# bifurcation/fourq

Hardware: NVIDIA B200
Metric: curve4q_variable_base_dh_scalar_mults_per_s (higher is better)
Workload: dtype u32

## Files before the change

### fourq_b200/csrc/codec.cuh

```cuda
#pragma once
#include "point.cuh"

#define FQ_ST_OK 0
#define FQ_ST_RESERVED_BIT 1
#define FQ_ST_NONCANONICAL 2
#define FQ_ST_QUIRK_T0 3
#define FQ_ST_NOT_ON_CURVE 4
#define FQ_ST_NEUTRAL 5

FQ_FN u32 pt_sign(const fp2& x) {
  u32 nz = x.re.v[0] | x.re.v[1] | x.re.v[2] | x.re.v[3];
  return (nz != 0) ? (x.re.v[3] >> 30) : (x.im.v[3] >> 30);
}

FQ_FN void pt_encode(const fp2& x, const fp2& y, u32* out) {
  FQ_UNROLL
  for (int i = 0; i < 4; i++) { out[i] = y.re.v[i]; out[4 + i] = y.im.v[i]; }
  out[7] |= pt_sign(x) << 31;
}

template <bool SPEC = false> FQ_FN u32 pt_decode(const u32* in, fp2& x, fp2& y) {
  u32 st = FQ_ST_OK;
  if (in[3] >> 31) st = FQ_ST_RESERVED_BIT;
  u32 s = in[7] >> 31;
  y.re = fp_set(in[0], in[1], in[2], in[3] & FQ_P3);
  y.im = fp_set(in[4], in[5], in[6], in[7] & FQ_P3);
  u32 y0p = in[0] & in[1] & in[2] & (in[3] | 0x80000000u);
  u32 y1p = in[4] & in[5] & in[6] & (in[7] | 0x80000000u);
  if (st == FQ_ST_OK && (y0p == 0xffffffffu || y1p == 0xffffffffu)) st = FQ_ST_NONCANONICAL;

  fp2 y2 = fp2_sqr_c(y);
  fp2 u = fp2_sub(y2, fp2_one());
  const fp2 dy2 = fp2_mul_c(curve_d(), y2);
  fp2 v = fp2_add(dy2, fp2_one());
  fpb V0 = fp_prep(v.re), V1 = fp_prep(v.im);
  fp t0 = fp_add(fp_mul_prep(u.re, V0), fp_mul_prep(u.im, V1));
  fp t1 = fp_sub(fp_mul_prep(u.im, V0), fp_mul_prep(u.re, V1));
  fp t2 = fp_add(fp_sqr(v.re), fp_sqr(v.im));
  fp t3 = fp_add(fp_sqr(t0), fp_sqr(t1));
  t3 = fp_mul(fp_invsqrt_c(t3), t3);
  fp t = fp_dbl(fp_add(t0, t3));
  if (SPEC) { if (fp_is_zero(t)) t = fp_dbl(fp_sub(t0, t3)); }
  else if (st == FQ_ST_OK && fp_is_zero(t)) st = FQ_ST_QUIRK_T0;
  fpb T2 = fp_prep(t2);
  fp a = fp_invsqrt_c(fp_mul(fp_mul_prep(fp_sqr(t2), T2), t));
  fp at2 = fp_mul_prep(a, T2);
  fp b = fp_mul(at2, t);
  fp x0 = fp_half(b);
  fp x1 = fp_mul(at2, t1);
  bool same = fp_eq_canon(fp_canon(t), fp_canon(fp_mul_prep(fp_sqr(b), T2)));
  u32 msw = same ? 0u : 0xffffffffu;
  x.re = fp_canon(fp_select(msw, x1, x0));
  x.im = fp_canon(fp_select(msw, x0, x1));
  u32 mneg = (pt_sign(x) != s) ? 0xffffffffu : 0u;
  x = fp2_canon(fp2_select(mneg, fp2_neg(x), x));
  y = fp2_canon(y);
  const fp2 x2 = fp2_sqr_c(x), x2c = fp2_conj(x2);
  bool on1 = fp2_eq(fp2_sub(y2, x2), fp2_add(fp2_one(), fp2_mul_c(dy2, x2)));
  fp2 xc = fp2_canon(fp2_conj(x));
  bool on2 = fp2_eq(fp2_sub(y2, x2c), fp2_add(fp2_one(), fp2_mul_c(dy2, x2c)));
  x = fp2_select(on1 ? 0xffffffffu : 0u, x, xc);
  if (st == FQ_ST_OK && !(on1 | on2)) st = FQ_ST_NOT_ON_CURVE;
  return st;
}
```

### fourq_b200/csrc/endo.cuh

```cuda
#pragma once
#include "dh.cuh"

FQ_FN fp2 endo_ctau() { return fp2_set(fp_set(0xebce74c3u, 0x74dcd57cu, 0x3afad20cu, 0x1964de2cu), fp_set(0x00000012u, 0x00000000u, 0x0000000cu, 0x00000000u)); }
FQ_FN fp2 endo_ctaudual() { return fp2_set(fp_set(0xdecdf034u, 0x9ecaa6d9u, 0x23058652u, 0x4aa740ebu), fp_set(0x00000011u, 0x00000000u, 0xfffffff4u, 0x7fffffffu)); }
FQ_FN fp2 endo_cphi0() { return fp2_set(fp_set(0xfffffff7u, 0xffffffffu, 0x00000005u, 0x00000000u), fp_set(0xef66f81au, 0x4f65536cu, 0x9182c329u, 0x2553a075u)); }
FQ_FN fp2 endo_cphi1() { return fp2_set(fp_set(0x00000007u, 0x00000000u, 0x00000005u, 0x00000000u), fp_set(0xe28296f9u, 0x334d90e9u, 0xc50c62cfu, 0x62c8caa0u)); }
FQ_FN fp2 endo_cphi2() { return fp2_set(fp_set(0x00000015u, 0x00000000u, 0x0000000fu, 0x00000000u), fp_set(0x4f1df391u, 0x2c2cb715u, 0x6c9b5c98u, 0x78df262bu)); }
FQ_FN fp2 endo_cphi3() { return fp2_set(fp_set(0x00000003u, 0x00000000u, 0x00000002u, 0x00000000u), fp_set(0xa7962ea4u, 0x92440457u, 0x1d76342au, 0x5084c649u)); }
FQ_FN fp2 endo_cphi4() { return fp2_set(fp_set(0x00000003u, 0x00000000u, 0x00000003u, 0x00000000u), fp_set(0x3aec6855u, 0xa1098c92u, 0xa7962ea4u, 0x12440457u)); }
FQ_FN fp2 endo_cphi5() { return fp2_set(fp_set(0x0000000fu, 0x00000000u, 0x0000000au, 0x00000000u), fp_set(0xc5052df3u, 0x669b21d3u, 0x8a18c59eu, 0x45919541u)); }
FQ_FN fp2 endo_cphi6() { return fp2_set(fp_set(0x00000018u, 0x00000000u, 0x00000012u, 0x00000000u), fp_set(0x8a0a5be7u, 0xcd3643a7u, 0x14318b3cu, 0x0b232a83u)); }
FQ_FN fp2 endo_cphi7() { return fp2_set(fp_set(0x00000023u, 0x00000000u, 0x00000018u, 0x00000000u), fp_set(0x5f48781au, 0x66c18303u, 0x99e2ea1au, 0x3963bc1cu)); }
FQ_FN fp2 endo_cphi8() { return fp2_set(fp_set(0x000000f0u, 0x00000000u, 0x000000aau, 0x00000000u), fp_set(0x2b5d0ef0u, 0x44e25158u, 0x0316cbe5u, 0x1f529f86u)); }
FQ_FN fp2 endo_cphi9() { return fp2_set(fp_set(0x00000befu, 0x00000000u, 0x00000870u, 0x00000000u), fp_set(0x976e2505u, 0x014d3e48u, 0xfe00375bu, 0x0fd52e9cu)); }
FQ_FN fp2 endo_cpsi1() { return fp2_set(fp_set(0x67e346efu, 0xedf07f47u, 0x83d54a02u, 0x2af99e9au), fp_set(0x0000013au, 0x00000000u, 0x000000deu, 0x00000000u)); }
FQ_FN fp2 endo_cpsi2() { return fp2_set(fp_set(0x00000143u, 0x00000000u, 0x000000e4u, 0x00000000u), fp_set(0x0e03f372u, 0x4c7deb77u, 0x99a81f03u, 0x21b8d07bu)); }
FQ_FN fp2 endo_cpsi3() { return fp2_set(fp_set(0x00000009u, 0x00000000u, 0x00000006u, 0x00000000u), fp_set(0x75e73a61u, 0x3a6e6abeu, 0x1d7d6906u, 0x4cb26f16u)); }
FQ_FN fp2 endo_cpsi4() { return fp2_set(fp_set(0xfffffff6u, 0xffffffffu, 0xfffffff9u, 0x7fffffffu), fp_set(0x8a18c59eu, 0xc5919541u, 0xe28296f9u, 0x334d90e9u)); }

struct pt3 { fp2 X, Y, Z; };

#if defined(FQ_ENDO_CALLS) && !defined(FQ_HOSTSIM)
#define FQ_ENDO_FN FQ_CALL
#else
#define FQ_ENDO_FN FQ_FN
#endif

FQ_FN fp2 fp2_two_sqr(const fp2& z) { return fp2_dbl(fp2_sqr_c(z)); }

FQ_ENDO_FN pt3 endo_tau(pt3 P) {
  fp2 A = fp2_sqr_c(P.X), B = fp2_sqr_c(P.Y);
  fp2 C = fp2_add(A, B), D = fp2_sub(A, B);
  pt3 R;
  R.X = fp2_mul_c(fp2_mul_c(fp2_mul_c(endo_ctau(), P.X), P.Y), D);
  R.Y = fp2_neg(fp2_mul_c(fp2_add(fp2_two_sqr(P.Z), D), C));
  R.Z = fp2_mul_c(C, D);
  return R;
}
FQ_ENDO_FN ptR1 endo_tau_dual(pt3 P) {
  fp2 A = fp2_sqr_c(P.X), B = fp2_sqr_c(P.Y);
  fp2 C = fp2_add(A, B);
  ptR1 R;
  R.Ta = fp2_sub(B, A);
  fp2 D = fp2_sub(fp2_two_sqr(P.Z), R.Ta);
  R.Tb = fp2_mul_c(fp2_mul_c(endo_ctaudual(), P.X), P.Y);
  R.X = fp2_mul_c(R.Tb, C); R.Y = fp2_mul_c(R.Ta, D); R.Z = fp2_mul_c(D, C);
  return R;
}
FQ_ENDO_FN pt3 endo_upsilon(pt3 P) {
  fp2 A = fp2_mul_c(fp2_mul_c(endo_cphi0(), P.X), P.Y);
  fp2 B = fp2_mul_c(P.Y, P.Z);
  fp2 C = fp2_sqr_c(P.Y), D = fp2_sqr_c(P.Z);
  fp2 F = fp2_sqr_c(D), G = fp2_sqr_c(B), H = fp2_sqr_c(C);
  fp2 I = fp2_mul_c(endo_cphi1(), B);
  fp2 J = fp2_add(C, fp2_mul_c(endo_cphi2(), D));
  fp2 K = fp2_add(fp2_add(fp2_mul_c(endo_cphi8(), G), H), fp2_mul_c(endo_cphi9(), F));
  pt3 R;
  R.X = fp2_conj(fp2_mul_c(fp2_mul_c(A, K), fp2_mul_c(fp2_add(I, J), fp2_sub(I, J))));
  fp2 L = fp2_add(C, fp2_mul_c(endo_cphi4(), D));
  fp2 M = fp2_mul_c(endo_cphi3(), B);
  fp2 Nn = fp2_mul_c(fp2_add(L, M), fp2_sub(L, M));
  fp2 Y2 = fp2_add(fp2_add(H, fp2_mul_c(endo_cphi6(), G)), fp2_mul_c(endo_cphi7(), F));
  R.Y = fp2_conj(fp2_mul_c(fp2_mul_c(fp2_mul_c(endo_cphi5(), D), Nn), Y2));
  R.Z = fp2_conj(fp2_mul_c(fp2_mul_c(B, K), Nn));
  return R;
}
FQ_ENDO_FN pt3 endo_chi(pt3 P) {
  fp2 A = fp2_conj(P.X), B = fp2_conj(P.Y);
  fp2 C = fp2_sqr_c(fp2_conj(P.Z));
  fp2 D = fp2_sqr_c(A);
  fp2 G = fp2_mul_c(B, fp2_add(D, fp2_mul_c(endo_cpsi2(), C)));
  fp2 H = fp2_neg(fp2_add(D, fp2_mul_c(endo_cpsi4(), C)));
  pt3 R;
  R.X = fp2_mul_c(fp2_mul_c(fp2_mul_c(endo_cpsi1(), A), C), H);
  R.Y = fp2_mul_c(G, fp2_add(D, fp2_mul_c(endo_cpsi3(), C)));
  R.Z = fp2_mul_c(G, H);
  return R;
}
FQ_FN pt3 pt3_of(const ptR1& P) { pt3 R; R.X = P.X; R.Y = P.Y; R.Z = P.Z; return R; }
FQ_FN ptR1 endo_phi(const ptR1& P) { return endo_tau_dual(endo_upsilon(endo_tau(pt3_of(P)))); }
FQ_FN ptR1 endo_psi(const ptR1& P) { return endo_tau_dual(endo_chi(endo_tau(pt3_of(P)))); }

FQ_CALL u64 endo_mulhi_256(u32 l0, u32 l1, u32 l2, u32 l3, u32 l4, u32 l5, u32 l6, scal m) {
  const u32 L[7] = {l0, l1, l2, l3, l4, l5, l6};
  u32 c0 = 0, c1 = 0, c2 = 0, out8 = 0, out9 = 0;
  FQ_UNROLL
  for (int k = 0; k < 10; k++) {
    FQ_UNROLL
    for (int i = 0; i < 7; i++) {
      const int j = k - i;
      if (j >= 0 && j < 8) { c0 = mad_lo_cc(L[i], m.v[j], c0); c1 = madc_hi_cc(L[i], m.v[j], c1); c2 = addc(c2, 0); }
    }
    if (k == 8) out8 = c0;
    if (k == 9) out9 = c0;
    c0 = c1; c1 = c2; c2 = 0;
  }
  return ((u64)out9 << 32) | out8;
}

struct scal4 { u64 v[4]; };

FQ_FN scal4 endo_decompose(const scal& m) {
  const u64 B1[4] = {0x0906ff27e0a0a196ull, 0xec9c179d3dd5d260ull, 0x07426031ecc8030full, 0xf7b08c66794619afull};
  const u64 B2[4] = {0x1d495bea84fcc2d4ull, 0xffffffffffffffffull, 0x0000000000000001ull, 0x25dbc5bc8dd167d0ull};
  const u64 B3[4] = {0x17abad1d231f0302ull, 0x02c4211ae388da51ull, 0xd1b2de3676d83b61ull, 0x0a9e6f44c02ecd97ull};
  const u64 B4[4] = {0x136e340a9108c83full, 0x3122df2dc3e0ff32ull, 0xf975b60fd557564bull, 0xe72af7876921f516ull};
  const u64 C[4] = {0x72482c5251a4559cull, 0x59f95b0add276f6cull, 0x7dd2d17c4625fa78ull, 0x6bc57def56ce8877ull};
  const u64 CP[4] = {0x85b6605ce2ad1ddbull, 0x8b1c3a38a1086e9eull, 0x7748878c1b7d50c3ull, 0x52f07576bff07d8dull};
  u64 t1 = endo_mulhi_256(0x9d1a7d4fu, 0x259686e0u, 0xe6a6bd66u, 0xf75682acu, 0xea2be5dfu, 0xfc5bb5c5u, 0x00000007u, m);
  u64 t2 = endo_mulhi_256(0xdd627afbu, 0xd1ba1d84u, 0x0f468d8du, 0x2bd23558u, 0xaa6c0f8au, 0x8fd4b04cu, 0x00000003u, m);
  u64 t3 = endo_mulhi_256(0x678c203cu, 0x9b291a33u, 0x65dca902u, 0xc42bd6c9u, 0x0bffbaf6u, 0xd038bf8du, 0x00000000u, m);
  u64 t4 = endo_mulhi_256(0x77e7fdc0u, 0x12e5666bu, 0x14983d82u, 0x81cbdc37u, 0xa22d8410u, 0x1b073877u, 0x00000003u, m);
  scal4 a;
  FQ_UNROLL
  for (int j = 0; j < 4; j++) {
    u64 x = (j == 0) ? (((u64)m.v[1] << 32) | m.v[0]) : 0ull;
    a.v[j] = x - t1 * B1[j] - t2 * B2[j] - t3 * B3[j] - t4 * B4[j];
  }
  u64 odd = 0ull - ((a.v[0] + C[0]) & 1ull);
  scal4 v;
  FQ_UNROLL
  for (int j = 0; j < 4; j++) v.v[j] = a.v[j] + ((C[j] & odd) | (CP[j] & ~odd));
  return v;
}

FQ_FN u32 endo_recode(const scal4& vin, scal& S) {
  u64 v0s = vin.v[0] >> 1, v1 = vin.v[1], v2 = vin.v[2], v3 = vin.v[3];
  FQ_UNROLL
  for (int w = 0; w < 8; w++) S.v[w] = 0;
  FQ_NOUNROLL
  for (int w = 0; w < 8; w++) {
    u32 word = 0;
    FQ_UNROLL
    for (int n = 0; n < 8; n++) {
      u32 b1 = (u32)(v0s & 1ull);
      v0s >>= 1;
      u32 e1 = (u32)(v1 & 1ull), e2 = (u32)(v2 & 1ull), e3 = (u32)(v3 & 1ull);
      word |= ((b1 << 3) | e1 | (e2 << 1) | (e3 << 2)) << (4 * n);
      u32 nb1 = b1 ^ 1u;
      v1 = (v1 >> 1) + (u64)(nb1 & e1); v2 = (v2 >> 1) + (u64)(nb1 & e2); v3 = (v3 >> 1) + (u64)(nb1 & e3);
    }
    FQ_UNROLL
    for (int i = 0; i < 7; i++) S.v[i] = S.v[i + 1];
    S.v[7] = word;
  }
  return (u32)(v1 + 2ull * v2 + 4ull * v3);
}
FQ_FN void endo_next_digit(scal& s, u32& idx, u32& neg) {
  u32 nib = s.v[7] >> 28;
  neg = (nib >> 3) - 1;
  idx = nib & 7;
  FQ_UNROLL
  for (int i = 7; i > 0; i--) s.v[i] = shl_pair(s.v[i - 1], s.v[i], 4);
  s.v[0] <<= 4;
}

FQ_FN ptR2 endo_tab_build(const TabView& T, const ptR1& P) {
  const pt3 tP = endo_tau(pt3_of(P));
  ptR1 Qp = endo_tau_dual(endo_upsilon(tP));
  ptR3 A3;
  ptR2 T0, Ti;
  ptR1 S;
  pt_r1_to_r2_c(&T0, &P);
  tab_store(T, 0, T0);
  pt_r1_to_r3_c(&A3, &Qp);
  pt_add_core_c(&S, &A3, &T0); pt_r1_to_r2_c(&Ti, &S); tab_store(T, 1, Ti);
  S = endo_tau_dual(endo_chi(tP));
  pt_r1_to_r3_c(&A3, &S);
  pt_add_core_c(&S, &A3, &Ti); pt_r1_to_r2_c(&Ti, &S); tab_store(T, 3, Ti);
  pt_add_core_c(&S, &A3, &T0); pt_r1_to_r2_c(&Ti, &S); tab_store(T, 2, Ti);
  S = endo_psi(Qp);
  pt_r1_to_r3_c(&A3, &S);
  FQ_NOUNROLL
  for (int i = 0; i < 4; i++) {
    Ti = tab_load(T, i);
    pt_add_core_c(&S, &A3, &Ti); pt_r1_to_r2_c(&Ti, &S);
    if (i < 3) tab_store(T, 4 + i, Ti);
  }
  return Ti;
}

FQ_FN MulPlan plan_endo(const scal& k) {
  MulPlan pl;
  pl.first = endo_recode(endo_decompose(k), pl.S);
  return pl;
}
template <class SELECT> FQ_FN ptR1 loop_endo(MulPlan& pl, SELECT select) {
  ptR1 Q = pt_r2_to_r4(select(pl.first));
  FQ_NOUNROLL
  for (int i = 63; i >= 0; i--) {
    pt_dbl(Q);
    u32 idx, neg;
    endo_next_digit(pl.S, idx, neg);
    Q = pt_add(Q, pt_r2_cneg(neg, select(idx)));
  }
  return Q;
}
template <class SELECT> FQ_FN ptR1 mul_endo(const scal& k, SELECT select) {
  MulPlan pl = plan_endo(k);
  return loop_endo(pl, select);
}

FQ_FN void dh_setup_endo(const scal& k, const fp2& x, const fp2& y, const TabView& T, DhState& D) {
  ptR1 Q = pt_clear_cofactor(x, y);
  D.T7 = endo_tab_build(T, Q);
  D.plan = plan_endo(k);
}
template <bool STRICT = FQ_STRICT_DEFAULT> FQ_FN ptR1 dh_loop_endo(const TabView& T, DhState& D) {
  SelectShared<STRICT> sel; sel.T = T; sel.T7 = D.T7;
  return loop_endo(D.plan, sel);
}
```

### fourq_b200/csrc/fp.cuh

```cuda
#pragma once
#include "arith.cuh"

struct fp { u32 v[4]; };

struct fpb { u32 b0, b1, b2, b3, e1, e2, e3, d2, d3; };

struct facc { u32 e0, e1, e2, e3, e4, o1, o2, o3, o4, o5; };

struct fpw { u32 w[6]; };

#define FQ_P3 0x7fffffffu

FQ_FN fp fp_set(u32 a0, u32 a1, u32 a2, u32 a3) { fp r; r.v[0] = a0; r.v[1] = a1; r.v[2] = a2; r.v[3] = a3; return r; }
FQ_FN fp fp_zero() { return fp_set(0, 0, 0, 0); }
FQ_FN fp fp_one() { return fp_set(1, 0, 0, 0); }


FQ_FN fp fp_add_loose(const fp& a, const fp& b) {
  fp r;
  r.v[0] = add_cc(a.v[0], b.v[0]); r.v[1] = addc_cc(a.v[1], b.v[1]);
  r.v[2] = addc_cc(a.v[2], b.v[2]); r.v[3] = addc(a.v[3], b.v[3]);
  return r;
}

FQ_FN fp fp_fold1(const fp& x) {
  fp r; u32 t = x.v[3] >> 31;
  r.v[0] = add_cc(x.v[0], t); r.v[1] = addc_cc(x.v[1], 0);
  r.v[2] = addc_cc(x.v[2], 0); r.v[3] = addc(x.v[3] & FQ_P3, 0);
  return r;
}

FQ_FN fp fp_add(const fp& a, const fp& b) { return fp_fold1(fp_add_loose(a, b)); }

FQ_FN fp fp_sub(const fp& a, const fp& b) {
  fp r;
  r.v[0] = sub_cc(a.v[0], b.v[0]); r.v[1] = subc_cc(a.v[1], b.v[1]);
  r.v[2] = subc_cc(a.v[2], b.v[2]); r.v[3] = subc_cc(a.v[3], b.v[3]);
  r.v[0] = subc_cc(r.v[0], 0); r.v[1] = subc_cc(r.v[1], 0);
  r.v[2] = subc_cc(r.v[2], 0); r.v[3] = subc(r.v[3], 0) & FQ_P3;
  return r;
}

FQ_FN fp fp_neg(const fp& a) { return fp_set(~a.v[0], ~a.v[1], ~a.v[2], a.v[3] ^ FQ_P3); }

FQ_FN fp fp_dbl(const fp& a) {
  return fp_set((a.v[0] << 1) | (a.v[3] >> 30), shl_pair(a.v[0], a.v[1], 1), shl_pair(a.v[1], a.v[2], 1),
                shl_pair(a.v[2], a.v[3], 1) & FQ_P3);
}
FQ_FN fp fp_half(const fp& a) {
  return fp_set(shr_pair(a.v[0], a.v[1], 1), shr_pair(a.v[1], a.v[2], 1), shr_pair(a.v[2], a.v[3], 1),
                (a.v[3] >> 1) | ((a.v[0] & 1) << 30));
}

FQ_FN fp fp_canon(const fp& a) {
  u32 allones = a.v[0] & a.v[1] & a.v[2] & (a.v[3] | 0x80000000u);
  u32 m = (allones == 0xffffffffu) ? 0u : 0xffffffffu;
  return fp_set(a.v[0] & m, a.v[1] & m, a.v[2] & m, a.v[3] & m);
}
FQ_FN bool fp_eq_canon(const fp& a, const fp& b) {
  return ((a.v[0] ^ b.v[0]) | (a.v[1] ^ b.v[1]) | (a.v[2] ^ b.v[2]) | (a.v[3] ^ b.v[3])) == 0;
}
FQ_FN bool fp_is_zero(const fp& a) {
  u32 o = a.v[0] | a.v[1] | a.v[2] | a.v[3];
  u32 n = a.v[0] & a.v[1] & a.v[2] & (a.v[3] | 0x80000000u);
  return (o == 0) | (n == 0xffffffffu);
}
FQ_FN fp fp_select(u32 m, const fp& x, const fp& y) {
  return fp_set(y.v[0] ^ (m & (x.v[0] ^ y.v[0])), y.v[1] ^ (m & (x.v[1] ^ y.v[1])),
                y.v[2] ^ (m & (x.v[2] ^ y.v[2])), y.v[3] ^ (m & (x.v[3] ^ y.v[3])));
}
FQ_FN fp fp_from_u128(const fp& x) { return fp_fold1(fp_fold1(x)); }


FQ_FN fpb fp_prep(const fp& b) {
  fpb B;
  B.b0 = b.v[0]; B.b1 = b.v[1]; B.b2 = b.v[2]; B.b3 = b.v[3];
  B.e1 = b.v[1] << 1; B.e2 = b.v[2] << 1; B.e3 = b.v[3] << 1;
  B.d2 = shl_pair(b.v[1], b.v[2], 1); B.d3 = shl_pair(b.v[2], b.v[3], 1);
  return B;
}

FQ_FN void facc_zero(facc& A) { A.e0 = A.e1 = A.e2 = A.e3 = A.e4 = A.o1 = A.o2 = A.o3 = A.o4 = A.o5 = 0; }

template <int K> FQ_FN void facc_init_kp(facc& A) {
  A.e0 = 0; A.e1 = 0u - (1u << (K - 32)); A.e2 = 0xffffffffu; A.e3 = 0xffffffffu; A.e4 = 0;
  A.o1 = 0; A.o2 = 0; A.o3 = 0; A.o4 = 0xffffffffu; A.o5 = (1u << (K - 33)) - 1u;
}

FQ_FN void facc_row0(facc& A, u32 a, u32 v0, u32 v1, u32 v2, u32 v3) {
  mul_wide(A.e0, A.e1, a, v0); mul_wide(A.e2, A.e3, a, v2); A.e4 = 0;
  mul_wide(A.o1, A.o2, a, v1); mul_wide(A.o3, A.o4, a, v3); A.o5 = 0;
}
FQ_FN void facc_row(facc& A, u32 a, u32 v0, u32 v1, u32 v2, u32 v3) {
  A.e0 = mad_lo_cc(a, v0, A.e0); A.e1 = madc_hi_cc(a, v0, A.e1);
  A.e2 = madc_lo_cc(a, v2, A.e2); A.e3 = madc_hi_cc(a, v2, A.e3); A.e4 = addc(A.e4, 0);
  A.o1 = mad_lo_cc(a, v1, A.o1); A.o2 = madc_hi_cc(a, v1, A.o2);
  A.o3 = madc_lo_cc(a, v3, A.o3); A.o4 = madc_hi_cc(a, v3, A.o4); A.o5 = addc(A.o5, 0);
}

template <bool FRESH> FQ_FN void facc_mul(facc& A, const fp& a, const fpb& B) {
  if (FRESH) facc_row0(A, a.v[0], B.b0, B.b1, B.b2, B.b3);
  else facc_row(A, a.v[0], B.b0, B.b1, B.b2, B.b3);
  facc_row(A, a.v[1], B.e3, B.b0, B.b1, B.b2);
  facc_row(A, a.v[2], B.e2, B.d3, B.b0, B.b1);
  facc_row(A, a.v[3], B.e1, B.d2, B.d3, B.b0);
}

FQ_FN fpw facc_merge(const facc& A) {
  fpw r;
  r.w[0] = A.e0; r.w[1] = add_cc(A.e1, A.o1); r.w[2] = addc_cc(A.e2, A.o2); r.w[3] = addc_cc(A.e3, A.o3);
  r.w[4] = addc_cc(A.e4, A.o4); r.w[5] = addc(A.o5, 0);
  return r;
}
FQ_FN fpw fpw_add(const fpw& a, const fpw& b) {
  fpw r;
  r.w[0] = add_cc(a.w[0], b.w[0]); r.w[1] = addc_cc(a.w[1], b.w[1]); r.w[2] = addc_cc(a.w[2], b.w[2]);
  r.w[3] = addc_cc(a.w[3], b.w[3]); r.w[4] = addc_cc(a.w[4], b.w[4]); r.w[5] = addc(a.w[5], b.w[5]);
  return r;
}
FQ_FN fpw fpw_sub(const fpw& a, const fpw& b) {
  fpw r;
  r.w[0] = sub_cc(a.w[0], b.w[0]); r.w[1] = subc_cc(a.w[1], b.w[1]); r.w[2] = subc_cc(a.w[2], b.w[2]);
  r.w[3] = subc_cc(a.w[3], b.w[3]); r.w[4] = subc_cc(a.w[4], b.w[4]); r.w[5] = subc(a.w[5], b.w[5]);
  return r;
}

FQ_FN fp fp_fold(const fpw& x) {
  fp r;
  u32 tlo = shr_pair(x.w[3], x.w[4], 31), thi = shr_pair(x.w[4], x.w[5], 31);
  r.v[0] = add_cc(x.w[0], tlo); r.v[1] = addc_cc(x.w[1], thi);
  r.v[2] = addc_cc(x.w[2], 0); r.v[3] = addc(x.w[3] & FQ_P3, 0);
  u32 top = r.v[3] >> 31;
  r.v[3] &= FQ_P3;
  r.v[0] = add_cc(r.v[0], top); r.v[1] = addc(r.v[1], 0);
  return r;
}

FQ_FN fp fp_mul_prep(const fp& a, const fpb& B) {
  facc A; facc_mul<true>(A, a, B);
  return fp_fold(facc_merge(A));
}
FQ_FN fp fp_mul(const fp& a, const fp& b) { return fp_mul_prep(a, fp_prep(b)); }
FQ_FN fp fp_fold7(u32 w0, u32 w1, u32 w2, u32 w3, u32 w4, u32 w5, u32 w6) {
  fp r;
  u32 t0 = shr_pair(w3, w4, 31), t1 = shr_pair(w4, w5, 31), t2 = shr_pair(w5, w6, 31), t3 = w6 >> 31;
  r.v[0] = add_cc(w0, t0); r.v[1] = addc_cc(w1, t1); r.v[2] = addc_cc(w2, t2); r.v[3] = addc(w3 & FQ_P3, t3);
  u32 top = r.v[3] >> 31;
  r.v[3] &= FQ_P3;
  r.v[0] = add_cc(r.v[0], top); r.v[1] = addc_cc(r.v[1], 0); r.v[2] = addc_cc(r.v[2], 0); r.v[3] = addc(r.v[3], 0);
  return r;
}
FQ_FN fp fp_sqr(const fp& a) {
  const u32 a0 = a.v[0], a1 = a.v[1], a2 = a.v[2], a3 = a.v[3];
  const u32 e1 = a1 << 1, e2 = a2 << 1, e3 = a3 << 1, d2 = shl_pair(a1, a2, 1), d3 = shl_pair(a2, a3, 1);
  u32 E0, E1, E2, E3, E4, E5, E6, O1, O2, O3, O4, O5, O6;
  mul_wide(E0, E1, a0, a0); mul_wide(E2, E3, a0, d2); mul_wide(E4, E5, a1, d3);
  E2 = mad_lo_cc(a1, a1, E2); E3 = madc_hi_cc(a1, a1, E3); E4 = madc_lo_cc(a2, a2, E4); E5 = madc_hi_cc(a2, a2, E5); E6 = addc(0, 0);
  E2 = mad_lo_cc(a3, e3, E2); E3 = madc_hi_cc(a3, e3, E3); E4 = addc_cc(E4, 0); E5 = addc_cc(E5, 0); E6 = addc(E6, 0);
  mul_wide(O1, O2, a0, e1); mul_wide(O3, O4, a0, d3); mul_wide(O5, O6, a2, e3);
  O3 = mad_lo_cc(a1, e2, O3); O4 = madc_hi_cc(a1, e2, O4); O5 = addc_cc(O5, 0); O6 = addc(O6, 0);
  u32 w1 = add_cc(E1, O1), w2 = addc_cc(E2, O2), w3 = addc_cc(E3, O3), w4 = addc_cc(E4, O4), w5 = addc_cc(E5, O5), w6 = addc(E6, O6);
  return fp_fold7(E0, w1, w2, w3, w4, w5, w6);
}

FQ_FN fp fp_nsqr(fp x, int n) {
  FQ_NOUNROLL
  for (int i = 0; i < n; i++) x = fp_sqr(x);
  return x;
}

FQ_FN fp fp_inv(const fp& x) {
  fp x3 = fp_mul(fp_sqr(x), x);
  fp xf = fp_mul(fp_nsqr(x3, 2), x3);
  fp x8 = fp_mul(fp_nsqr(xf, 4), xf);
  fp x16 = fp_mul(fp_nsqr(x8, 8), x8);
  fp x32 = fp_mul(fp_nsqr(x16, 16), x16);
  fp t = fp_mul(fp_nsqr(x32, 32), x32);
  t = fp_mul(fp_nsqr(t, 32), x32);
  t = fp_mul(fp_nsqr(t, 16), x16);
  t = fp_mul(fp_nsqr(t, 8), x8);
  t = fp_mul(fp_nsqr(t, 4), xf);
  t = fp_mul(fp_sqr(t), x);
  return fp_mul(fp_nsqr(t, 2), x);
}

FQ_FN fp fp_invsqrt(const fp& x) {
  fp x3 = fp_mul(fp_sqr(x), x);
  fp xf = fp_mul(fp_nsqr(x3, 2), x3);
  fp x5 = fp_mul(fp_sqr(xf), x);
  fp x10 = fp_mul(fp_nsqr(x5, 5), x5);
  fp x20 = fp_mul(fp_nsqr(x10, 10), x10);
  fp x25 = fp_mul(fp_nsqr(x20, 5), x5);
  fp x50 = fp_mul(fp_nsqr(x25, 25), x25);
  fp x100 = fp_mul(fp_nsqr(x50, 50), x50);
  fp x125 = fp_mul(fp_nsqr(x100, 25), x25);
  return x125;
}
```

### fourq_b200/csrc/fp2.cuh

```cuda
#pragma once
#include "fp.cuh"

struct fp2 { fp re, im; };

struct fp2b { fpb re, im, sum; };

FQ_FN fp2 fp2_set(const fp& re, const fp& im) { fp2 r; r.re = re; r.im = im; return r; }
FQ_FN fp2 fp2_zero() { return fp2_set(fp_zero(), fp_zero()); }
FQ_FN fp2 fp2_one() { return fp2_set(fp_one(), fp_zero()); }

FQ_FN fp2 fp2_add(const fp2& a, const fp2& b) { return fp2_set(fp_add(a.re, b.re), fp_add(a.im, b.im)); }
FQ_FN fp2 fp2_sub(const fp2& a, const fp2& b) { return fp2_set(fp_sub(a.re, b.re), fp_sub(a.im, b.im)); }
FQ_FN fp2 fp2_neg(const fp2& a) { return fp2_set(fp_neg(a.re), fp_neg(a.im)); }
FQ_FN fp2 fp2_conj(const fp2& a) { return fp2_set(a.re, fp_neg(a.im)); }
FQ_FN fp2 fp2_dbl(const fp2& a) { return fp2_set(fp_dbl(a.re), fp_dbl(a.im)); }
FQ_FN fp2 fp2_canon(const fp2& a) { return fp2_set(fp_canon(a.re), fp_canon(a.im)); }
FQ_FN bool fp2_eq_canon(const fp2& a, const fp2& b) { return fp_eq_canon(a.re, b.re) & fp_eq_canon(a.im, b.im); }
FQ_FN bool fp2_eq(const fp2& a, const fp2& b) { return fp2_eq_canon(fp2_canon(a), fp2_canon(b)); }
FQ_FN fp2 fp2_select(u32 m, const fp2& x, const fp2& y) { return fp2_set(fp_select(m, x.re, y.re), fp_select(m, x.im, y.im)); }

#ifdef FQ_FP2_SCHOOLBOOK
FQ_FN fp2b fp2_prep(const fp2& b) {
  fp2b B;
  B.re = fp_prep(b.re); B.im = fp_prep(b.im); B.sum = B.re;
  return B;
}
FQ_FN fp2 fp2_mul_prep(const fp2& a, const fp2b& B) {
  facc A0, A1;
  facc_mul<true>(A0, a.re, B.re); facc_mul<false>(A0, fp_neg(a.im), B.im);
  facc_mul<true>(A1, a.re, B.im); facc_mul<false>(A1, a.im, B.re);
  fp2 r;
  r.re = fp_fold(facc_merge(A0));
  r.im = fp_fold(facc_merge(A1));
  return r;
}
#else
FQ_FN fp2b fp2_prep(const fp2& b) {
  fp2b B;
  B.re = fp_prep(b.re); B.im = fp_prep(b.im); B.sum = fp_prep(fp_add(b.re, b.im));
  return B;
}

FQ_FN fp2 fp2_mul_prep(const fp2& a, const fp2b& B) {
  facc A0, A1, A2;
  facc_init_kp<36>(A0); facc_mul<false>(A0, a.re, B.re);
  facc_mul<true>(A1, a.im, B.im);
  facc_init_kp<38>(A2); facc_mul<false>(A2, fp_add_loose(a.re, a.im), B.sum);
  fpw t0 = facc_merge(A0), t1 = facc_merge(A1), t2 = facc_merge(A2);
  fp2 r;
  r.re = fp_fold(fpw_sub(t0, t1));
  r.im = fp_fold(fpw_sub(fpw_sub(t2, t0), t1));
  return r;
}
#endif
FQ_FN fp2 fp2_mul(const fp2& a, const fp2& b) { return fp2_mul_prep(a, fp2_prep(b)); }

FQ_FN fp2 fp2_sqr(const fp2& a) {
  fp2 r;
  r.re = fp_mul_prep(fp_add_loose(a.re, a.im), fp_prep(fp_sub(a.re, a.im)));
  r.im = fp_mul_prep(fp_add_loose(a.re, a.re), fp_prep(a.im));
  return r;
}

FQ_FN fp2 fp2_inv(const fp2& a) {
  fp n = fp_inv(fp_add(fp_sqr(a.re), fp_sqr(a.im)));
  fpb N = fp_prep(n);
  return fp2_set(fp_mul_prep(a.re, N), fp_mul_prep(fp_neg(a.im), N));
}

#ifdef FQ_HOSTSIM
#define FQ_CALL static inline
#else
#define FQ_CALL static __device__ __noinline__
#endif
FQ_CALL fp2 fp2_mul_c(fp2 a, fp2 b) { return fp2_mul(a, b); }
FQ_CALL fp2 fp2_sqr_c(fp2 a) { return fp2_sqr(a); }
FQ_CALL fp fp_invsqrt_c(fp a) { return fp_invsqrt(a); }
```

### fourq_b200/csrc/point.cuh

```cuda
#pragma once
#include "fp2.cuh"

struct ptR1 { fp2 X, Y, Z, Ta, Tb; };
struct ptR2 { fp2 N, D, E, F; };
struct ptR3p { fp2b N, D, E, F; };

FQ_FN fp2 curve_d() { return fp2_set(fp_set(0x00000142u, 0x00000000u, 0x000000e4u, 0x00000000u), fp_set(0xf1fc0c8du, 0xb3821488u, 0x6657e0fcu, 0x5e472f84u)); }
FQ_FN fp2 curve_2d() { return fp2_set(fp_set(0x00000284u, 0x00000000u, 0x000001c8u, 0x00000000u), fp_set(0xe3f8191bu, 0x67042911u, 0xccafc1f9u, 0x3c8e5f08u)); }
FQ_FN fp2 curve_gx() { return fp2_set(fp_set(0x7b3833aau, 0x286592adu, 0x7c2fb305u, 0x1a347223u), fp_set(0x60ac77f6u, 0x96869fb3u, 0x2878aa9cu, 0x1e1f553fu)); }
FQ_FN fp2 curve_gy() { return fp2_set(fp_set(0x2bcbb287u, 0xb924a246u, 0xa120785au, 0x0e3fee9bu), fp_set(0x844c8b5cu, 0x49a7c344u, 0x630e0242u, 0x6e1c4af8u)); }

FQ_CALL bool pt_on_curve(fp2 x, fp2 y) {
  fp2 x2 = fp2_sqr_c(x), y2 = fp2_sqr_c(y);
  fp2 lhs = fp2_sub(y2, x2);
  fp2 rhs = fp2_add(fp2_one(), fp2_mul_c(fp2_mul_c(curve_d(), x2), y2));
  return fp2_eq(lhs, rhs);
}

FQ_FN ptR1 pt_from_affine(const fp2& x, const fp2& y) { ptR1 P; P.X = x; P.Y = y; P.Z = fp2_one(); P.Ta = x; P.Tb = y; return P; }

FQ_FN ptR2 pt_r1_to_r2(const ptR1& P) {
  ptR2 R;
  R.N = fp2_add(P.X, P.Y); R.D = fp2_sub(P.Y, P.X); R.E = fp2_dbl(P.Z);
  R.F = fp2_mul(fp2_mul(P.Ta, P.Tb), curve_2d());
  return R;
}
FQ_FN ptR3p pt_r1_to_r3p(const ptR1& P) {
  ptR3p R;
  R.N = fp2_prep(fp2_add(P.X, P.Y)); R.D = fp2_prep(fp2_sub(P.Y, P.X)); R.E = fp2_prep(P.Z);
  R.F = fp2_prep(fp2_mul(P.Ta, P.Tb));
  return R;
}
FQ_FN ptR1 pt_r2_to_r4(const ptR2& P) {
  ptR1 Q; Q.X = fp2_sub(P.N, P.D); Q.Y = fp2_add(P.D, P.N); Q.Z = P.E; Q.Ta = fp2_zero(); Q.Tb = fp2_zero();
  return Q;
}
FQ_FN ptR2 pt_r2_cneg(u32 m, const ptR2& P) {
  ptR2 R;
  R.N = fp2_select(m, P.D, P.N); R.D = fp2_select(m, P.N, P.D); R.E = P.E;
  R.F.re = fp_set(P.F.re.v[0] ^ m, P.F.re.v[1] ^ m, P.F.re.v[2] ^ m, P.F.re.v[3] ^ (m & FQ_P3));
  R.F.im = fp_set(P.F.im.v[0] ^ m, P.F.im.v[1] ^ m, P.F.im.v[2] ^ m, P.F.im.v[3] ^ (m & FQ_P3));
  return R;
}

FQ_FN void pt_dbl(ptR1& Q) {
  fp2 A = fp2_sqr(Q.X); FQ_SCHED_FENCE();
  fp2 B = fp2_sqr(Q.Y); FQ_SCHED_FENCE();
  fp2 C = fp2_dbl(fp2_sqr(Q.Z)); FQ_SCHED_FENCE();
  fp2 D = fp2_add(A, B);
  fp2 E = fp2_sub(fp2_sqr(fp2_add(Q.X, Q.Y)), D); FQ_SCHED_FENCE();
  fp2 F = fp2_sub(B, A);
  fp2 G = fp2_sub(C, F);
  fp2b Gp = fp2_prep(G), Fp = fp2_prep(F);
  Q.X = fp2_mul_prep(E, Gp); FQ_SCHED_FENCE();
  Q.Y = fp2_mul_prep(D, Fp); FQ_SCHED_FENCE();
  Q.Z = fp2_mul_prep(F, Gp); FQ_SCHED_FENCE();
  Q.Ta = E; Q.Tb = D;
}

FQ_FN ptR1 pt_add_core(const ptR3p& P, const ptR2& S) {
  fp2 A = fp2_mul_prep(S.D, P.D); FQ_SCHED_FENCE();
  fp2 B = fp2_mul_prep(S.N, P.N); FQ_SCHED_FENCE();
  fp2 C = fp2_mul_prep(S.F, P.F); FQ_SCHED_FENCE();
  fp2 D = fp2_mul_prep(S.E, P.E); FQ_SCHED_FENCE();
  fp2 E = fp2_sub(B, A), F = fp2_sub(D, C), G = fp2_add(D, C), H = fp2_add(B, A);
  fp2b Fp = fp2_prep(F), Gp = fp2_prep(G);
  ptR1 R;
  R.X = fp2_mul_prep(E, Fp); FQ_SCHED_FENCE();
  R.Y = fp2_mul_prep(H, Gp); FQ_SCHED_FENCE();
  R.Z = fp2_mul_prep(G, Fp); FQ_SCHED_FENCE();
  R.Ta = E; R.Tb = H;
  return R;
}
FQ_FN ptR1 pt_add(const ptR1& Q, const ptR2& S) { return pt_add_core(pt_r1_to_r3p(Q), S); }

struct ptR3 { fp2 N, D, E, F; };
#ifdef FQ_SMALL_POINT_OPS
FQ_CALL ptR1 pt_dbl_v(ptR1 Q) {
  fp2 A = fp2_sqr_c(Q.X), B = fp2_sqr_c(Q.Y), C = fp2_dbl(fp2_sqr_c(Q.Z));
  fp2 D = fp2_add(A, B), E = fp2_sub(fp2_sqr_c(fp2_add(Q.X, Q.Y)), D), F = fp2_sub(B, A), G = fp2_sub(C, F);
  ptR1 R; R.X = fp2_mul_c(E, G); R.Y = fp2_mul_c(D, F); R.Z = fp2_mul_c(F, G); R.Ta = E; R.Tb = D;
  return R;
}
#else
FQ_CALL ptR1 pt_dbl_v(ptR1 q) { pt_dbl(q); return q; }
#endif
FQ_FN void pt_dbl_c(ptR1* Q) { *Q = pt_dbl_v(*Q); }
FQ_FN void pt_r1_to_r3_c(ptR3* R, const ptR1* P) {
  R->N = fp2_add(P->X, P->Y); R->D = fp2_sub(P->Y, P->X); R->E = P->Z; R->F = fp2_mul_c(P->Ta, P->Tb);
}
#ifdef FQ_SMALL_POINT_OPS
FQ_CALL ptR1 pt_add_core_v(ptR3 P, ptR2 S) {
  fp2 A = fp2_mul_c(S.D, P.D), B = fp2_mul_c(S.N, P.N), C = fp2_mul_c(S.F, P.F), D = fp2_mul_c(S.E, P.E);
  fp2 E = fp2_sub(B, A), F = fp2_sub(D, C), G = fp2_add(D, C), H = fp2_add(B, A);
  ptR1 R; R.X = fp2_mul_c(E, F); R.Y = fp2_mul_c(H, G); R.Z = fp2_mul_c(G, F); R.Ta = E; R.Tb = H;
  return R;
}
#else
FQ_CALL ptR1 pt_add_core_v(ptR3 P, ptR2 S) {
  ptR3p Pp; Pp.N = fp2_prep(P.N); Pp.D = fp2_prep(P.D); Pp.E = fp2_prep(P.E); Pp.F = fp2_prep(P.F);
  return pt_add_core(Pp, S);
}
#endif
FQ_FN void pt_add_core_c(ptR1* out, const ptR3* P, const ptR2* S) { *out = pt_add_core_v(*P, *S); }
FQ_FN void pt_r1_to_r2_c(ptR2* R, const ptR1* P) {
  R->N = fp2_add(P->X, P->Y); R->D = fp2_sub(P->Y, P->X); R->E = fp2_dbl(P->Z);
  R->F = fp2_mul_c(fp2_mul_c(P->Ta, P->Tb), curve_2d());
}

FQ_FN ptR1 pt_clear_cofactor(const fp2& x, const fp2& y) {
  ptR1 Q = pt_from_affine(x, y);
  ptR2 B; pt_r1_to_r2_c(&B, &Q);
  FQ_NOUNROLL
  for (int i = 0; i < 10; i++) {
    if (i == 1 || i == 6) { ptR3 Q3; pt_r1_to_r3_c(&Q3, &Q); pt_add_core_c(&Q, &Q3, &B); }
    else pt_dbl_c(&Q);
  }
  return Q;
}

FQ_FN void pt_to_affine(const ptR1& P, fp2& x, fp2& y) {
  fp2b Zi = fp2_prep(fp2_inv(P.Z));
  x = fp2_canon(fp2_mul_prep(P.X, Zi)); y = fp2_canon(fp2_mul_prep(P.Y, Zi));
}
```

Before: 91.26 million.

## Specialize multiplication by curve and endomorphism constants with short limbs

Adds a templated fp2 constant multiplier that exploits constants whose one component is a small value of the form s0 + s2*2^64, replacing a full limb product with a few narrow multiply-adds. All curve-d, 2d and endomorphism constant multiplications in decode, endomorphisms, table construction and on-curve checks now go through it. It also partially unrolls the repeated squaring loops in inverse square root by two. This cuts integer multiply work in precomputation, at the cost of more template instantiations and code size.

```diff
diff --git a/fourq_b200/csrc/codec.cuh b/fourq_b200/csrc/codec.cuh
--- a/fourq_b200/csrc/codec.cuh
+++ b/fourq_b200/csrc/codec.cuh
@@ -31,7 +31,7 @@
 
   fp2 y2 = fp2_sqr_c(y);
   fp2 u = fp2_sub(y2, fp2_one());
-  const fp2 dy2 = fp2_mul_c(curve_d(), y2);
+  const fp2 dy2 = fp2_mul_k<curve_dk>(y2);
   fp2 v = fp2_add(dy2, fp2_one());
   fpb V0 = fp_prep(v.re), V1 = fp_prep(v.im);
   fp t0 = fp_add(fp_mul_prep(u.re, V0), fp_mul_prep(u.im, V1));
diff --git a/fourq_b200/csrc/endo.cuh b/fourq_b200/csrc/endo.cuh
--- a/fourq_b200/csrc/endo.cuh
+++ b/fourq_b200/csrc/endo.cuh
@@ -1,22 +1,22 @@
 #pragma once
 #include "dh.cuh"
 
-FQ_FN fp2 endo_ctau() { return fp2_set(fp_set(0xebce74c3u, 0x74dcd57cu, 0x3afad20cu, 0x1964de2cu), fp_set(0x00000012u, 0x00000000u, 0x0000000cu, 0x00000000u)); }
-FQ_FN fp2 endo_ctaudual() { return fp2_set(fp_set(0xdecdf034u, 0x9ecaa6d9u, 0x23058652u, 0x4aa740ebu), fp_set(0x00000011u, 0x00000000u, 0xfffffff4u, 0x7fffffffu)); }
-FQ_FN fp2 endo_cphi0() { return fp2_set(fp_set(0xfffffff7u, 0xffffffffu, 0x00000005u, 0x00000000u), fp_set(0xef66f81au, 0x4f65536cu, 0x9182c329u, 0x2553a075u)); }
-FQ_FN fp2 endo_cphi1() { return fp2_set(fp_set(0x00000007u, 0x00000000u, 0x00000005u, 0x00000000u), fp_set(0xe28296f9u, 0x334d90e9u, 0xc50c62cfu, 0x62c8caa0u)); }
-FQ_FN fp2 endo_cphi2() { return fp2_set(fp_set(0x00000015u, 0x00000000u, 0x0000000fu, 0x00000000u), fp_set(0x4f1df391u, 0x2c2cb715u, 0x6c9b5c98u, 0x78df262bu)); }
-FQ_FN fp2 endo_cphi3() { return fp2_set(fp_set(0x00000003u, 0x00000000u, 0x00000002u, 0x00000000u), fp_set(0xa7962ea4u, 0x92440457u, 0x1d76342au, 0x5084c649u)); }
-FQ_FN fp2 endo_cphi4() { return fp2_set(fp_set(0x00000003u, 0x00000000u, 0x00000003u, 0x00000000u), fp_set(0x3aec6855u, 0xa1098c92u, 0xa7962ea4u, 0x12440457u)); }
-FQ_FN fp2 endo_cphi5() { return fp2_set(fp_set(0x0000000fu, 0x00000000u, 0x0000000au, 0x00000000u), fp_set(0xc5052df3u, 0x669b21d3u, 0x8a18c59eu, 0x45919541u)); }
-FQ_FN fp2 endo_cphi6() { return fp2_set(fp_set(0x00000018u, 0x00000000u, 0x00000012u, 0x00000000u), fp_set(0x8a0a5be7u, 0xcd3643a7u, 0x14318b3cu, 0x0b232a83u)); }
-FQ_FN fp2 endo_cphi7() { return fp2_set(fp_set(0x00000023u, 0x00000000u, 0x00000018u, 0x00000000u), fp_set(0x5f48781au, 0x66c18303u, 0x99e2ea1au, 0x3963bc1cu)); }
-FQ_FN fp2 endo_cphi8() { return fp2_set(fp_set(0x000000f0u, 0x00000000u, 0x000000aau, 0x00000000u), fp_set(0x2b5d0ef0u, 0x44e25158u, 0x0316cbe5u, 0x1f529f86u)); }
-FQ_FN fp2 endo_cphi9() { return fp2_set(fp_set(0x00000befu, 0x00000000u, 0x00000870u, 0x00000000u), fp_set(0x976e2505u, 0x014d3e48u, 0xfe00375bu, 0x0fd52e9cu)); }
-FQ_FN fp2 endo_cpsi1() { return fp2_set(fp_set(0x67e346efu, 0xedf07f47u, 0x83d54a02u, 0x2af99e9au), fp_set(0x0000013au, 0x00000000u, 0x000000deu, 0x00000000u)); }
-FQ_FN fp2 endo_cpsi2() { return fp2_set(fp_set(0x00000143u, 0x00000000u, 0x000000e4u, 0x00000000u), fp_set(0x0e03f372u, 0x4c7deb77u, 0x99a81f03u, 0x21b8d07bu)); }
-FQ_FN fp2 endo_cpsi3() { return fp2_set(fp_set(0x00000009u, 0x00000000u, 0x00000006u, 0x00000000u), fp_set(0x75e73a61u, 0x3a6e6abeu, 0x1d7d6906u, 0x4cb26f16u)); }
-FQ_FN fp2 endo_cpsi4() { return fp2_set(fp_set(0xfffffff6u, 0xffffffffu, 0xfffffff9u, 0x7fffffffu), fp_set(0x8a18c59eu, 0xc5919541u, 0xe28296f9u, 0x334d90e9u)); }
+typedef fp2k<false, 0xebce74c3u, 0x74dcd57cu, 0x3afad20cu, 0x1964de2cu, 0x12, 0xc> endo_ctau;
+typedef fp2k<false, 0xdecdf034u, 0x9ecaa6d9u, 0x23058652u, 0x4aa740ebu, 0x12, -0xc> endo_ctaudual;
+typedef fp2k<true, 0xef66f81au, 0x4f65536cu, 0x9182c329u, 0x2553a075u, -0x9, 0x6> endo_cphi0;
+typedef fp2k<true, 0xe28296f9u, 0x334d90e9u, 0xc50c62cfu, 0x62c8caa0u, 0x7, 0x5> endo_cphi1;
+typedef fp2k<true, 0x4f1df391u, 0x2c2cb715u, 0x6c9b5c98u, 0x78df262bu, 0x15, 0xf> endo_cphi2;
+typedef fp2k<true, 0xa7962ea4u, 0x92440457u, 0x1d76342au, 0x5084c649u, 0x3, 0x2> endo_cphi3;
+typedef fp2k<true, 0x3aec6855u, 0xa1098c92u, 0xa7962ea4u, 0x12440457u, 0x3, 0x3> endo_cphi4;
+typedef fp2k<true, 0xc5052df3u, 0x669b21d3u, 0x8a18c59eu, 0x45919541u, 0xf, 0xa> endo_cphi5;
+typedef fp2k<true, 0x8a0a5be7u, 0xcd3643a7u, 0x14318b3cu, 0x0b232a83u, 0x18, 0x12> endo_cphi6;
+typedef fp2k<true, 0x5f48781au, 0x66c18303u, 0x99e2ea1au, 0x3963bc1cu, 0x23, 0x18> endo_cphi7;
+typedef fp2k<true, 0x2b5d0ef0u, 0x44e25158u, 0x0316cbe5u, 0x1f529f86u, 0xf0, 0xaa> endo_cphi8;
+typedef fp2k<true, 0x976e2505u, 0x014d3e48u, 0xfe00375bu, 0x0fd52e9cu, 0xbef, 0x870> endo_cphi9;
+typedef fp2k<false, 0x67e346efu, 0xedf07f47u, 0x83d54a02u, 0x2af99e9au, 0x13a, 0xde> endo_cpsi1;
+typedef fp2k<true, 0x0e03f372u, 0x4c7deb77u, 0x99a81f03u, 0x21b8d07bu, 0x143, 0xe4> endo_cpsi2;
+typedef fp2k<true, 0x75e73a61u, 0x3a6e6abeu, 0x1d7d6906u, 0x4cb26f16u, 0x9, 0x6> endo_cpsi3;
+typedef fp2k<true, 0x8a18c59eu, 0xc5919541u, 0xe28296f9u, 0x334d90e9u, -0x9, -0x6> endo_cpsi4;
 
 struct pt3 { fp2 X, Y, Z; };
 
@@ -32,7 +32,7 @@
   fp2 A = fp2_sqr_c(P.X), B = fp2_sqr_c(P.Y);
   fp2 C = fp2_add(A, B), D = fp2_sub(A, B);
   pt3 R;
-  R.X = fp2_mul_c(fp2_mul_c(fp2_mul_c(endo_ctau(), P.X), P.Y), D);
+  R.X = fp2_mul_c(fp2_mul_c(fp2_mul_k<endo_ctau>(P.X), P.Y), D);
   R.Y = fp2_neg(fp2_mul_c(fp2_add(fp2_two_sqr(P.Z), D), C));
   R.Z = fp2_mul_c(C, D);
   return R;
@@ -43,25 +43,25 @@
   ptR1 R;
   R.Ta = fp2_sub(B, A);
   fp2 D = fp2_sub(fp2_two_sqr(P.Z), R.Ta);
-  R.Tb = fp2_mul_c(fp2_mul_c(endo_ctaudual(), P.X), P.Y);
+  R.Tb = fp2_mul_c(fp2_mul_k<endo_ctaudual>(P.X), P.Y);
   R.X = fp2_mul_c(R.Tb, C); R.Y = fp2_mul_c(R.Ta, D); R.Z = fp2_mul_c(D, C);
   return R;
 }
 FQ_ENDO_FN pt3 endo_upsilon(pt3 P) {
-  fp2 A = fp2_mul_c(fp2_mul_c(endo_cphi0(), P.X), P.Y);
+  fp2 A = fp2_mul_c(fp2_mul_k<endo_cphi0>(P.X), P.Y);
   fp2 B = fp2_mul_c(P.Y, P.Z);
   fp2 C = fp2_sqr_c(P.Y), D = fp2_sqr_c(P.Z);
   fp2 F = fp2_sqr_c(D), G = fp2_sqr_c(B), H = fp2_sqr_c(C);
-  fp2 I = fp2_mul_c(endo_cphi1(), B);
-  fp2 J = fp2_add(C, fp2_mul_c(endo_cphi2(), D));
-  fp2 K = fp2_add(fp2_add(fp2_mul_c(endo_cphi8(), G), H), fp2_mul_c(endo_cphi9(), F));
+  fp2 I = fp2_mul_k<endo_cphi1>(B);
+  fp2 J = fp2_add(C, fp2_mul_k<endo_cphi2>(D));
+  fp2 K = fp2_add(fp2_add(fp2_mul_k<endo_cphi8>(G), H), fp2_mul_k<endo_cphi9>(F));
   pt3 R;
   R.X = fp2_conj(fp2_mul_c(fp2_mul_c(A, K), fp2_mul_c(fp2_add(I, J), fp2_sub(I, J))));
-  fp2 L = fp2_add(C, fp2_mul_c(endo_cphi4(), D));
-  fp2 M = fp2_mul_c(endo_cphi3(), B);
+  fp2 L = fp2_add(C, fp2_mul_k<endo_cphi4>(D));
+  fp2 M = fp2_mul_k<endo_cphi3>(B);
   fp2 Nn = fp2_mul_c(fp2_add(L, M), fp2_sub(L, M));
-  fp2 Y2 = fp2_add(fp2_add(H, fp2_mul_c(endo_cphi6(), G)), fp2_mul_c(endo_cphi7(), F));
-  R.Y = fp2_conj(fp2_mul_c(fp2_mul_c(fp2_mul_c(endo_cphi5(), D), Nn), Y2));
+  fp2 Y2 = fp2_add(fp2_add(H, fp2_mul_k<endo_cphi6>(G)), fp2_mul_k<endo_cphi7>(F));
+  R.Y = fp2_conj(fp2_mul_c(fp2_mul_c(fp2_mul_k<endo_cphi5>(D), Nn), Y2));
   R.Z = fp2_conj(fp2_mul_c(fp2_mul_c(B, K), Nn));
   return R;
 }
@@ -69,11 +69,11 @@
   fp2 A = fp2_conj(P.X), B = fp2_conj(P.Y);
   fp2 C = fp2_sqr_c(fp2_conj(P.Z));
   fp2 D = fp2_sqr_c(A);
-  fp2 G = fp2_mul_c(B, fp2_add(D, fp2_mul_c(endo_cpsi2(), C)));
-  fp2 H = fp2_neg(fp2_add(D, fp2_mul_c(endo_cpsi4(), C)));
+  fp2 G = fp2_mul_c(B, fp2_add(D, fp2_mul_k<endo_cpsi2>(C)));
+  fp2 H = fp2_neg(fp2_add(D, fp2_mul_k<endo_cpsi4>(C)));
   pt3 R;
-  R.X = fp2_mul_c(fp2_mul_c(fp2_mul_c(endo_cpsi1(), A), C), H);
-  R.Y = fp2_mul_c(G, fp2_add(D, fp2_mul_c(endo_cpsi3(), C)));
+  R.X = fp2_mul_c(fp2_mul_c(fp2_mul_k<endo_cpsi1>(A), C), H);
+  R.Y = fp2_mul_c(G, fp2_add(D, fp2_mul_k<endo_cpsi3>(C)));
   R.Z = fp2_mul_c(G, H);
   return R;
 }
diff --git a/fourq_b200/csrc/fp.cuh b/fourq_b200/csrc/fp.cuh
--- a/fourq_b200/csrc/fp.cuh
+++ b/fourq_b200/csrc/fp.cuh
@@ -163,9 +163,14 @@
   return fp_fold7(E0, w1, w2, w3, w4, w5, w6);
 }
 
-FQ_FN fp fp_nsqr(fp x, int n) {
+template <int U = 1> FQ_FN fp fp_nsqr(fp x, int n) {
+  FQ_UNROLL
+  for (int i = 0; i < n % U; i++) x = fp_sqr(x);
   FQ_NOUNROLL
-  for (int i = 0; i < n; i++) x = fp_sqr(x);
+  for (int i = 0; i < n / U; i++) {
+    FQ_UNROLL
+    for (int j = 0; j < U; j++) x = fp_sqr(x);
+  }
   return x;
 }
 
@@ -186,13 +191,13 @@
 
 FQ_FN fp fp_invsqrt(const fp& x) {
   fp x3 = fp_mul(fp_sqr(x), x);
-  fp xf = fp_mul(fp_nsqr(x3, 2), x3);
+  fp xf = fp_mul(fp_nsqr<2>(x3, 2), x3);
   fp x5 = fp_mul(fp_sqr(xf), x);
-  fp x10 = fp_mul(fp_nsqr(x5, 5), x5);
-  fp x20 = fp_mul(fp_nsqr(x10, 10), x10);
-  fp x25 = fp_mul(fp_nsqr(x20, 5), x5);
-  fp x50 = fp_mul(fp_nsqr(x25, 25), x25);
-  fp x100 = fp_mul(fp_nsqr(x50, 50), x50);
-  fp x125 = fp_mul(fp_nsqr(x100, 25), x25);
+  fp x10 = fp_mul(fp_nsqr<2>(x5, 5), x5);
+  fp x20 = fp_mul(fp_nsqr<2>(x10, 10), x10);
+  fp x25 = fp_mul(fp_nsqr<2>(x20, 5), x5);
+  fp x50 = fp_mul(fp_nsqr<2>(x25, 25), x25);
+  fp x100 = fp_mul(fp_nsqr<2>(x50, 50), x50);
+  fp x125 = fp_mul(fp_nsqr<2>(x100, 25), x25);
   return x125;
 }
diff --git a/fourq_b200/csrc/fp2.cuh b/fourq_b200/csrc/fp2.cuh
--- a/fourq_b200/csrc/fp2.cuh
+++ b/fourq_b200/csrc/fp2.cuh
@@ -76,3 +76,42 @@
 FQ_CALL fp2 fp2_mul_c(fp2 a, fp2 b) { return fp2_mul(a, b); }
 FQ_CALL fp2 fp2_sqr_c(fp2 a) { return fp2_sqr(a); }
 FQ_CALL fp fp_invsqrt_c(fp a) { return fp_invsqrt(a); }
+
+template <bool SHORT_RE, u32 F0, u32 F1, u32 F2, u32 F3, int S0, int S2> struct fp2k {
+  static constexpr bool short_re = SHORT_RE;
+  static constexpr u32 f0 = F0, f1 = F1, f2 = F2, f3 = F3;
+  static constexpr int s0 = S0, s2 = S2;
+  static FQ_MFN fp2 value() {
+    const __int128 P = (__int128)(((unsigned __int128)1 << 127) - 1);
+    __int128 v = (__int128)S0 + (__int128)S2 * (__int128)(((unsigned __int128)1) << 64);
+    if (v < 0) v += P;
+    const fp s = fp_set((u32)v, (u32)(v >> 32), (u32)(v >> 64), (u32)(v >> 96)), f = fp_set(F0, F1, F2, F3);
+    return SHORT_RE ? fp2_set(s, f) : fp2_set(f, s);
+  }
+};
+
+template <int S0, int S2> FQ_FN void facc_short(facc& A, const fp& a, const fp& na) {
+  const fp& x = S0 < 0 ? na : a;
+  const fp& y = S2 < 0 ? na : a;
+  const u32 u0 = (u32)(S0 < 0 ? -S0 : S0), u2 = (u32)(S2 < 0 ? -S2 : S2), v2 = 2 * u2;
+  mul_wide(A.e0, A.e1, x.v[0], u0); mul_wide(A.e2, A.e3, x.v[2], u0);
+  A.e0 = mad_lo_cc(y.v[2], v2, A.e0); A.e1 = madc_hi_cc(y.v[2], v2, A.e1);
+  A.e2 = madc_lo_cc(y.v[0], u2, A.e2); A.e3 = madc_hi_cc(y.v[0], u2, A.e3); A.e4 = addc(0, 0);
+  mul_wide(A.o1, A.o2, x.v[1], u0); mul_wide(A.o3, A.o4, x.v[3], u0);
+  A.o1 = mad_lo_cc(y.v[3], v2, A.o1); A.o2 = madc_hi_cc(y.v[3], v2, A.o2);
+  A.o3 = madc_lo_cc(y.v[1], u2, A.o3); A.o4 = madc_hi_cc(y.v[1], u2, A.o4); A.o5 = addc(0, 0);
+}
+
+template <class K> FQ_CALL fp2 fp2_mul_k(fp2 a) {
+  const fpb F = fp_prep(fp_set(K::f0, K::f1, K::f2, K::f3));
+  const fp nre = fp_neg(a.re), nim = fp_neg(a.im);
+  facc A0, A1;
+  if (K::short_re) {
+    facc_short<K::s0, K::s2>(A0, a.re, nre); facc_mul<false>(A0, nim, F);
+    facc_short<K::s0, K::s2>(A1, a.im, nim); facc_mul<false>(A1, a.re, F);
+  } else {
+    facc_short<K::s0, K::s2>(A0, nim, a.im); facc_mul<false>(A0, a.re, F);
+    facc_short<K::s0, K::s2>(A1, a.re, nre); facc_mul<false>(A1, a.im, F);
+  }
+  return fp2_set(fp_fold(facc_merge(A0)), fp_fold(facc_merge(A1)));
+}
diff --git a/fourq_b200/csrc/point.cuh b/fourq_b200/csrc/point.cuh
--- a/fourq_b200/csrc/point.cuh
+++ b/fourq_b200/csrc/point.cuh
@@ -5,15 +5,16 @@
 struct ptR2 { fp2 N, D, E, F; };
 struct ptR3p { fp2b N, D, E, F; };
 
-FQ_FN fp2 curve_d() { return fp2_set(fp_set(0x00000142u, 0x00000000u, 0x000000e4u, 0x00000000u), fp_set(0xf1fc0c8du, 0xb3821488u, 0x6657e0fcu, 0x5e472f84u)); }
-FQ_FN fp2 curve_2d() { return fp2_set(fp_set(0x00000284u, 0x00000000u, 0x000001c8u, 0x00000000u), fp_set(0xe3f8191bu, 0x67042911u, 0xccafc1f9u, 0x3c8e5f08u)); }
+typedef fp2k<true, 0xf1fc0c8du, 0xb3821488u, 0x6657e0fcu, 0x5e472f84u, 0x142, 0xe4> curve_dk;
+typedef fp2k<true, 0xe3f8191bu, 0x67042911u, 0xccafc1f9u, 0x3c8e5f08u, 0x284, 0x1c8> curve_2dk;
+FQ_FN fp2 curve_2d() { return curve_2dk::value(); }
 FQ_FN fp2 curve_gx() { return fp2_set(fp_set(0x7b3833aau, 0x286592adu, 0x7c2fb305u, 0x1a347223u), fp_set(0x60ac77f6u, 0x96869fb3u, 0x2878aa9cu, 0x1e1f553fu)); }
 FQ_FN fp2 curve_gy() { return fp2_set(fp_set(0x2bcbb287u, 0xb924a246u, 0xa120785au, 0x0e3fee9bu), fp_set(0x844c8b5cu, 0x49a7c344u, 0x630e0242u, 0x6e1c4af8u)); }
 
 FQ_CALL bool pt_on_curve(fp2 x, fp2 y) {
   fp2 x2 = fp2_sqr_c(x), y2 = fp2_sqr_c(y);
   fp2 lhs = fp2_sub(y2, x2);
-  fp2 rhs = fp2_add(fp2_one(), fp2_mul_c(fp2_mul_c(curve_d(), x2), y2));
+  fp2 rhs = fp2_add(fp2_one(), fp2_mul_c(fp2_mul_k<curve_dk>(x2), y2));
   return fp2_eq(lhs, rhs);
 }
 
@@ -105,7 +106,7 @@
 FQ_FN void pt_add_core_c(ptR1* out, const ptR3* P, const ptR2* S) { *out = pt_add_core_v(*P, *S); }
 FQ_FN void pt_r1_to_r2_c(ptR2* R, const ptR1* P) {
   R->N = fp2_add(P->X, P->Y); R->D = fp2_sub(P->Y, P->X); R->E = fp2_dbl(P->Z);
-  R->F = fp2_mul_c(fp2_mul_c(P->Ta, P->Tb), curve_2d());
+  R->F = fp2_mul_k<curve_2dk>(fp2_mul_c(P->Ta, P->Tb));
 }
 
 FQ_FN ptR1 pt_clear_cofactor(const fp2& x, const fp2& y) {
```

Result: no change. 91.65 million (median of 6 runs) (+0.4%).
